# MaxChen228/pingpong-selfplay-ai

Hardware: AMD Instinct MI355X
Metric: env-steps/sec (whole node) at 65536 arenas, 1/2/4/8 GPUs; CPU-ref baseline (higher is better)
Workload: dtype f64 env state / f32 QNet; 1 GPU; configs[2]: 65536 arenas/GPU, full DQN train_iterative loop (act both players + env tick + PER push/sample + double-DQN update + Adam + target sync); arenas_per_gpu=65536, global_arenas=65536, pool=8, batch=256, updates_per_vector_step=1, memory_size=1000000, parallelism=dp1 (arena shards, 1 all-reduce/update)

## Files before the change

### pingpong-selfplay-ai_amd/csrc/pm_mfma.h

```cpp
#pragma once
#include "pm_dev.h"

namespace pm {

typedef float f32x16 __attribute__((ext_vector_type(16)));
typedef float f32x4v16 __attribute__((ext_vector_type(4)));
typedef __attribute__((address_space(3))) void lds_void;

constexpr int PLAIN = 4936;
enum : int {
    F_W1 = 0,
    F_W2 = 512,
    F_B1 = 4608,
    F_B2 = 4672,
    F_H = 4736,
    F_BH = 4992,
    F_SIZE = 5008,
};
static_assert(PLAIN + F_SIZE == PM_QNET_NW, "effective weight block size");

__device__ __forceinline__ int rho(int r) { return (r & 3) + 8 * (r >> 2); }

__device__ __forceinline__ float relu(float x) { return __int_as_float(max(__float_as_int(x), 0)); }

__device__ __forceinline__ void write_feature_frag_image(const float* __restrict__ p, float* __restrict__ f) {
    const int t = threadIdx.x, nt = blockDim.x;
    for (int k = t; k < 512; k += nt) {
        const int jt = k >> 8, lane = (k >> 2) & 63, s = k & 3;
        const int row = 32 * jt + (lane & 31), kk = 2 * s + (lane >> 5);
        f[F_W1 + k] = kk == 0 ? p[B1 + row] : p[W1 + row * 7 + kk - 1];
    }
    for (int k = t; k < 4096; k += nt) {
        const int e = k & 3, lane = (k >> 2) & 63, rq = (k >> 8) & 3, tt = (k >> 10) & 1, jt = k >> 11;
        const int row = 32 * jt + (lane & 31), col = 32 * tt + rho(4 * rq + e) + 4 * (lane >> 5);
        f[F_W2 + k] = p[W2 + row * 64 + col];
    }
    for (int k = t; k < 64; k += nt) {
        const int r = k & 15, h = (k >> 4) & 1, jt = k >> 5;
        f[F_B1 + k] = p[B1 + 32 * jt + rho(r) + 4 * h];
        f[F_B2 + k] = p[B2 + 32 * jt + rho(r) + 4 * h];
    }
}
__device__ __forceinline__ void write_feature_frags(const float* __restrict__ p, float* __restrict__ w) {
    for (int k = threadIdx.x; k < PM_QNET_HEAD_OFF; k += blockDim.x) w[k] = p[k];
    write_feature_frag_image(p, w + PLAIN);
}

__device__ __forceinline__ void write_head_frags(const float* heads, float* __restrict__ w) {
    const int t = threadIdx.x, nt = blockDim.x;
    for (int k = t; k < 260; k += nt) w[WH + k] = heads[k];
    float* f = w + PLAIN;
    for (int k = t; k < 256; k += nt) {
        const int c = k & 3, r = (k >> 2) & 15, tt = (k >> 6) & 1, h = k >> 7;
        f[F_H + k] = heads[c * 64 + 32 * tt + rho(r) + 4 * h];
    }
    if (t < 16) f[F_BH + t] = t < 4 ? heads[256 + t] : 0.f;
}

constexpr int kLwChunks = (F_SIZE / 4 + 63) / 64;
constexpr int kLwFloats = kLwChunks * 256;

template <int N>
__device__ __forceinline__ void copy_lds_f32(const float* __restrict__ src, float* dst) {
    const int wv = threadIdx.x >> 6, lane = threadIdx.x & 63, nw = blockDim.x >> 6;
    for (int c = wv; c * 64 < N; c += nw) {
        const int k = min(c * 64 + lane, N - 1);
        __builtin_amdgcn_global_load_lds((const void*)(src + k), (lds_void*)(dst + c * 64), 4, 0, 0);
    }
}
constexpr int pad64(int n) { return (n + 63) / 64 * 64; }
template <int N>
__device__ __forceinline__ void copy_lds_f32x4(const float* __restrict__ src, float* dst) {
    static_assert(N % 4 == 0, "whole float4s");
    const int wv = threadIdx.x >> 6, lane = threadIdx.x & 63, nw = blockDim.x >> 6;
    const float4* s4 = reinterpret_cast<const float4*>(src);
    for (int c = wv; c * 256 < N; c += nw) {
        const int k = min(c * 64 + lane, N / 4 - 1);
        __builtin_amdgcn_global_load_lds((const void*)(s4 + k), (lds_void*)(dst + c * 256), 16, 0, 0);
    }
}
constexpr int pad256(int n) { return (n + 255) / 256 * 256; }

__device__ __forceinline__ void stage_frags_lds(const float* __restrict__ w, float* lw, int rot) {
    const int wv = threadIdx.x >> 6, lane = threadIdx.x & 63, nw = blockDim.x >> 6;
    const float4* src = reinterpret_cast<const float4*>(w + PLAIN);
    float4* lw4 = reinterpret_cast<float4*>(lw);
    rot %= kLwChunks;
    for (int c0 = wv; c0 < kLwChunks; c0 += nw) {
        const int c = c0 + rot < kLwChunks ? c0 + rot : c0 + rot - kLwChunks;
        const int k = min(c * 64 + lane, F_SIZE / 4 - 1);
        __builtin_amdgcn_global_load_lds((const void*)(src + k), (lds_void*)(lw4 + c * 64), 16, 0, 0);
    }
}

constexpr int kListNets = 64;
constexpr int kListBlock = 256;
struct OppListSmem {
    int woff[kListBlock / 64][kListNets];
    int noff[kListNets], ncnt[kListNets];
};
__device__ __forceinline__ void write_opp_lists(int nn, int32_t* opp_list, int32_t* opp_cnt, OppListSmem& sm, int blk,
                                                int i, bool valid, int net) {
    if (nn > kListNets) return;
    const int lane = threadIdx.x & 63, wv = threadIdx.x >> 6;
    int rank = 0;
    for (int k = 0; k < nn; ++k) {
        const bool m = valid && net == k;
        const unsigned long long b = __ballot(m);
        if (m) rank = __popcll(b & ((1ull << lane) - 1ull));
        if (lane == 0) sm.woff[wv][k] = __popcll(b);
    }
    __syncthreads();
    if (wv == 0) {
        int acc = 0;
        if (lane < nn) {
            for (int w = 0; w < kListBlock / 64; ++w) {
                const int c = sm.woff[w][lane];
                sm.woff[w][lane] = acc;
                acc += c;
            }
        }
        const int inc = wave_incl_scan_i32(acc);
        if (lane < nn) { sm.ncnt[lane] = acc; sm.noff[lane] = inc - acc; }
    }
    __syncthreads();
    if (valid) opp_list[(size_t)blk * kListBlock + sm.noff[net] + sm.woff[wv][net] + rank] = i;
    if ((int)threadIdx.x < nn) opp_cnt[(size_t)blk * nn + threadIdx.x] = (sm.noff[threadIdx.x] << 16) | sm.ncnt[threadIdx.x];
}

__device__ __forceinline__ void compact_load(const int32_t* __restrict__ id, int lo, int hi, int (&v)[16]) {
    const int base = lo + 16 * (int)threadIdx.x;
    if (base + 16 <= hi && (reinterpret_cast<uintptr_t>(id + base) & 15) == 0) {
        const int4* p4 = reinterpret_cast<const int4*>(id + base);
#pragma unroll
        for (int q = 0; q < 4; ++q) {
            const int4 x = p4[q];
            v[4 * q] = x.x; v[4 * q + 1] = x.y; v[4 * q + 2] = x.z; v[4 * q + 3] = x.w;
        }
    } else {
#pragma unroll
        for (int r = 0; r < 16; ++r) v[r] = base + r < hi ? id[base + r] : -1;
    }
}
__device__ __forceinline__ void compact_scan(const int (&v)[16], int net, int lo, int* list, int* count, int* wtot) {
    const int t = threadIdx.x, lane = t & 63, wv = t >> 6, nw = blockDim.x >> 6;
    const int base = lo + 16 * t;
    unsigned mask = 0;
#pragma unroll
    for (int r = 0; r < 16; ++r) mask |= (v[r] == net ? 1u : 0u) << r;
    const int c = __popc(mask);
    const int incl = wave_incl_scan_i32(c);
    if (lane == 63) wtot[wv] = incl;
    __syncthreads();
    int off = 0, total = 0;
    for (int w = 0; w < nw; ++w) {
        off += w < wv ? wtot[w] : 0;
        total += wtot[w];
    }
    int p = off + incl - c;
    while (mask) {
        const int r = __ffs(mask) - 1;
        mask &= mask - 1;
        list[p++] = base + r;
    }
    if (t == 0) *count = total;
}

struct TileOut {
    int8_t* act;
    float* q;
    double eps;
    uint64_t seed, ctr;
};

__device__ __forceinline__ void heads_to_frags(const float* heads, float* hf) {
    for (int k = threadIdx.x; k < 260; k += blockDim.x) {
        if (k < 256) {
            const int c = k & 3, r = (k >> 2) & 15, tt = (k >> 6) & 1, h = k >> 7;
            hf[k] = heads[c * 64 + 32 * tt + rho(r) + 4 * h];
        } else {
            hf[k] = heads[k];
        }
    }
}

__device__ __forceinline__ void tile_hidden_h1(const float* lw, const float (&xs)[4], int lane, f32x16 (&c1)[2],
                                               f32x16 (&c2)[2]) {
    const int h = lane >> 5;
    const f32x16 zero = {};
#pragma unroll
    for (int jt = 0; jt < 2; ++jt) {
        const float4 w = reinterpret_cast<const float4*>(lw + F_W1)[jt * 64 + lane];
        c1[jt] = __builtin_amdgcn_mfma_f32_32x32x2f32(w.x, xs[0], zero, 0, 0, 0);
        c1[jt] = __builtin_amdgcn_mfma_f32_32x32x2f32(w.y, xs[1], c1[jt], 0, 0, 0);
        c1[jt] = __builtin_amdgcn_mfma_f32_32x32x2f32(w.z, xs[2], c1[jt], 0, 0, 0);
        c1[jt] = __builtin_amdgcn_mfma_f32_32x32x2f32(w.w, xs[3], c1[jt], 0, 0, 0);
    }
#pragma unroll
    for (int jt = 0; jt < 2; ++jt)
#pragma unroll
        for (int r = 0; r < 16; ++r) c1[jt][r] = relu(c1[jt][r]);
    const float4* w2 = reinterpret_cast<const float4*>(lw + F_W2) + lane;
#pragma unroll
    for (int jt = 0; jt < 2; ++jt) {
        const float4* b = reinterpret_cast<const float4*>(lw + F_B2 + (jt * 2 + h) * 16);
#pragma unroll
        for (int q4 = 0; q4 < 4; ++q4) {
            const float4 v = b[q4];
            c2[jt][4 * q4 + 0] = v.x; c2[jt][4 * q4 + 1] = v.y; c2[jt][4 * q4 + 2] = v.z; c2[jt][4 * q4 + 3] = v.w;
        }
    }
    float4 wcur = w2[0];
#pragma unroll
    for (int g8 = 0; g8 < 16; ++g8) {
        const int jt = g8 >> 3, t = (g8 >> 2) & 1, rq = g8 & 3;
        const float4 wnext = w2[((g8 + 1) & 15) * 64];
        c2[jt] = __builtin_amdgcn_mfma_f32_32x32x2f32(wcur.x, c1[t][4 * rq + 0], c2[jt], 0, 0, 0);
        c2[jt] = __builtin_amdgcn_mfma_f32_32x32x2f32(wcur.y, c1[t][4 * rq + 1], c2[jt], 0, 0, 0);
        c2[jt] = __builtin_amdgcn_mfma_f32_32x32x2f32(wcur.z, c1[t][4 * rq + 2], c2[jt], 0, 0, 0);
        c2[jt] = __builtin_amdgcn_mfma_f32_32x32x2f32(wcur.w, c1[t][4 * rq + 3], c2[jt], 0, 0, 0);
        wcur = wnext;
        __builtin_amdgcn_sched_barrier(0);
    }
}
__device__ __forceinline__ void tile_hidden(const float* lw, const float (&xs)[4], int lane, f32x16 (&c2)[2]) {
    f32x16 c1[2];
    tile_hidden_h1(lw, xs, lane, c1, c2);
}

__device__ __forceinline__ void tile_heads(const float* hf, const f32x16 (&c2)[2], int lane, float (&q)[3]) {
    const int h = lane >> 5;
    float v = 0.f, a0 = 0.f, a1 = 0.f, a2 = 0.f;
    const float4* hw = reinterpret_cast<const float4*>(hf + h * 128);
#pragma unroll
    for (int t = 0; t < 2; ++t) {
#pragma unroll
        for (int r = 0; r < 16; ++r) {
            const float x = relu(c2[t][r]);
            const float4 w = hw[t * 16 + r];
            v = fmaf(w.x, x, v);
            a0 = fmaf(w.y, x, a0);
            a1 = fmaf(w.z, x, a1);
            a2 = fmaf(w.w, x, a2);
        }
        __builtin_amdgcn_sched_barrier(0);
    }
    v += __shfl_xor(v, 32);
    a0 += __shfl_xor(a0, 32);
    a1 += __shfl_xor(a1, 32);
    a2 += __shfl_xor(a2, 32);
    v += hf[256];
    a0 += hf[257];
    a1 += hf[258];
    a2 += hf[259];
    const float mean = ((a0 + a1) + a2) / 3.0f;
    q[0] = v + (a0 - mean);
    q[1] = v + (a1 - mean);
// ... 375 lines not shown
```

### pingpong-selfplay-ai_amd/csrc/pm_per.h

```cpp
#pragma once
#include <hip/hip_runtime.h>
#include <stdint.h>

#include "pongmi.h"
#include "pm_dev.h"

namespace pm {

constexpr int PER_SUB = 64;
constexpr int PER_FAN = 16;
constexpr int PER_CHUNK = PER_SUB * PER_FAN;

__host__ __device__ inline int64_t per_pad(int64_t n_doubles) { return ((n_doubles * 8 + 255) / 256) * 256; }

struct PerTree {
    double* chunk;
    double* sub;
    float* leaf;
    int64_t nchunk, nsub;
};

__host__ __device__ inline PerTree per_tree(void* work, int64_t cap) {
    PerTree t;
    t.nsub = (cap + PER_SUB - 1) / PER_SUB;
// ... 131 lines not shown
        int64_t d = d0 + i;
        if (d >= pr.cap) d -= pr.cap;
        acc += lo + i < pr.cap ? (double)(d < pr.n ? pr.pval : v[i]) : 0.0;
    }
    return acc;
}
__device__ __forceinline__ double per_combine(double q0, double q1, double q2, double q3) {
    return ((q0 + q1) + q2) + q3;
}
__device__ __forceinline__ double per_sub_sum(const float* __restrict__ leaf, int64_t sb, const PushRange pr) {
    const double q0 = per_quarter(leaf, sb, 0, pr), q1 = per_quarter(leaf, sb, 1, pr);
    const double q2 = per_quarter(leaf, sb, 2, pr), q3 = per_quarter(leaf, sb, 3, pr);
    return per_combine(q0, q1, q2, q3);
}
__device__ __forceinline__ double per_sub_sum4(const float* __restrict__ leaf, int64_t sb, const PushRange pr) {
    const int lane = threadIdx.x & 63;
    const double q = per_quarter(leaf, sb, lane & 3, pr);
    return per_combine(quad_f64<0>(q), quad_f64<1>(q), quad_f64<2>(q), quad_f64<3>(q));
}

__device__ __forceinline__ bool per_sub_pushed(int64_t sb, const PushRange pr) {
    const int64_t lo = sb * PER_SUB;
    return lo + PER_SUB <= pr.cap && pr.dist(lo) + PER_SUB <= pr.n;
}
__device__ __forceinline__ double per_sub_pushed_sum(const PushRange pr) {
    double q = 0.0;
#pragma unroll
    for (int i = 0; i < 16; ++i) q += (double)pr.pval;
    return per_combine(q, q, q, q);
}

__device__ __forceinline__ double per_chunk_sum(const PerTree& t, int64_t c) {
    double v[PER_FAN];
#pragma unroll
    for (int k = 0; k < PER_FAN; ++k) v[k] = c * PER_FAN + k < t.nsub ? t.sub[c * PER_FAN + k] : 0.0;
    double acc = 0.0;
#pragma unroll
    for (int k = 0; k < PER_FAN; ++k) acc += v[k];
    return acc;
}

__device__ __forceinline__ void per_nodes_block(const PerTree& tr, const PushRange& pr, double* subl) {
    const int64_t sb = (int64_t)blockIdx.x * 64 + (threadIdx.x >> 2);
    const double v = per_sub_sum4(tr.leaf, sb < tr.nsub ? sb : tr.nsub - 1, pr);
    if ((threadIdx.x & 3) == 0) {
        subl[threadIdx.x >> 2] = sb < tr.nsub ? v : 0.0;
        if (sb < tr.nsub) tr.sub[sb] = v;
    }
    __syncthreads();
    const int64_t c = (int64_t)blockIdx.x * 4 + threadIdx.x;
    if (threadIdx.x < 4 && c < tr.nchunk) {
        double acc = 0.0;
#pragma unroll
        for (int k = 0; k < PER_FAN; ++k) acc += subl[threadIdx.x * PER_FAN + k];
        tr.chunk[c] = acc;
    }
}

constexpr int PER_BS = 64;
constexpr int PER_ROUND = 1024;

struct PerSampleSmem {
    double incl[PER_ROUND];
    double wsum[4];
};

__device__ inline double per_round_prefix(const double (&v)[4], double base, PerSampleSmem& sm) {
    const int t = threadIdx.x, lane = t & 63, wv = t >> 6;
    double run[4], acc = 0.0;
#pragma unroll
    for (int e = 0; e < 4; ++e) { acc += v[e]; run[e] = acc; }
    const double incl = wave_incl_scan_dpp(acc, lane);
    const double excl = wave_shr1_f64(incl);
    if (lane == 63) sm.wsum[wv] = incl;
    __syncthreads();
    double wb = base;
    for (int w = 0; w < wv; ++w) wb += sm.wsum[w];
    const double ex = wb + excl;
#pragma unroll
    for (int e = 0; e < 4; ++e) sm.incl[4 * t + e] = ex + run[e];
    const double tot = ((base + sm.wsum[0]) + sm.wsum[1]) + sm.wsum[2] + sm.wsum[3];
    __syncthreads();
    return tot;
}

__device__ __forceinline__ int per_lds_search(const PerSampleSmem& sm, int n, double x) {
    static_assert(PER_ROUND == 1024, "per_lds_search's five base-4 digits");
    int base = 0;
#pragma unroll
    for (int stride = 256; stride >= 1; stride >>= 2) {
        const int np = stride == 256 ? 4 : 3;
        double v[4];
#pragma unroll
        for (int i = 0; i < np; ++i) v[i] = sm.incl[min(base + stride * (i + 1) - 1, n - 1)];
        int cnt = 0;
#pragma unroll
        for (int i = 0; i < np; ++i) cnt += (base + stride * (i + 1) - 1 < n && !(v[i] > x)) ? 1 : 0;
        base += stride * cnt;
    }
    return base;
}

template <int NV>
__device__ __forceinline__ int per_group_find(const double (&v)[NV], double x, double& before, double& val) {
    const int lane = threadIdx.x & 63, q = lane & 3, g0 = lane & ~3;
    double acc = 0.0;
#pragma unroll
    for (int e = 0; e < NV; ++e) acc += v[e];
    const double s0 = quad_f64<0>(acc), s1 = quad_f64<1>(acc), s2 = quad_f64<2>(acc);
    const double ex = q == 0 ? 0.0 : (q == 1 ? s0 : (q == 2 ? s0 + s1 : (s0 + s1) + s2));
    double pre[NV + 1];
    pre[0] = ex;
#pragma unroll
    for (int e = 0; e < NV; ++e) pre[e + 1] = pre[e] + v[e];
    int k = -1;
    double hb = 0.0, hv = 0.0;
#pragma unroll
    for (int e = NV - 1; e >= 0; --e) {
        const bool h = pre[e + 1] > x;
        k = h ? e : k;
        hb = h ? pre[e] : hb;
        hv = h ? v[e] : hv;
    }
    const unsigned gh = (unsigned)(__ballot(k >= 0) >> g0) & 15u;
    int src;
    if (gh) {
        src = __ffs(gh) - 1;
    } else {
        hb = ex;
        hv = 0.0;
#pragma unroll
        for (int e = 0; e < NV; ++e) {
            const bool z = v[e] > 0.0;
            k = z ? e : k;
            hb = z ? pre[e] : hb;
            hv = z ? v[e] : hv;
        }
        const unsigned gn = (unsigned)(__ballot(k >= 0) >> g0) & 15u;
        src = gn ? 31 - __clz(gn) : 0;
        k = k < 0 ? 0 : k;
    }
    const int kk = quad_sel_i32(k, src);
    before = quad_sel_f64(hb, src);
    val = quad_sel_f64(hv, src);
    return src * NV + kk;
}

struct NoHook {
    __device__ void operator()() const {}
};
__device__ __forceinline__ float per_is_weight(int64_t size, double pa, double total, double beta) {
    return (float)pow((double)size * (pa / total), -beta);
}
template <bool RAW = false, class UFn, class OutFn, class Hook = NoHook>
__device__ inline void per_sample_block(bool active, int64_t size, const PerTree& tr, const PushRange& pr, double beta,
                                        int j0, int bs, PerSampleSmem& sm, UFn ufn, OutFn out, Hook l2done = Hook()) {
    const int t = threadIdx.x, q = t & 3;
    const int j = j0 + (t >> 2);
    const bool one_round = tr.nchunk <= PER_ROUND;
    double vc[4] = {0.0, 0.0, 0.0, 0.0};
    if (one_round) {
#pragma unroll
        for (int e = 0; e < 4; ++e) {
            const int64_t c = 4 * t + e;
            vc[e] = c < tr.nchunk ? tr.chunk[c] : 0.0;
        }
        asm volatile("" ::"v"(vc[0]), "v"(vc[1]), "v"(vc[2]), "v"(vc[3]));
    }
    if (!active) return;
    const int64_t nb = (size + PER_CHUNK - 1) / PER_CHUNK;
    const double u = j < bs ? ufn(j) : 0.0;
    double total = 0.0;
    if (nb > PER_ROUND) {
        for (int64_t c0 = 0; c0 < nb; c0 += PER_ROUND) {
            double v[4];
#pragma unroll
            for (int e = 0; e < 4; ++e) {
                const int64_t c = c0 + 4 * t + e;
                v[e] = c < nb ? tr.chunk[c] : 0.0;
            }
            total = per_round_prefix(v, total, sm);
        }
    }
    int64_t blk = -1, lastnz = 0;
    double before = 0.0, lastbef = 0.0, x = 0.0, run = 0.0;
    for (int64_t c0 = 0; c0 < nb; c0 += PER_ROUND) {
        double v[4];
#pragma unroll
        for (int e = 0; e < 4; ++e) {
            const int64_t c = c0 + 4 * t + e;
            v[e] = c < nb ? (one_round ? vc[e] : tr.chunk[c]) : 0.0;
        }
        const double end = per_round_prefix(v, run, sm);
        if (nb <= PER_ROUND) total = end;
        x = u * total;
        const int n = (int)(nb - c0 < PER_ROUND ? nb - c0 : PER_ROUND);
        if (blk < 0 && end > run) {
            const int k = per_lds_search(sm, n, x);
            if (k < n) {
                blk = c0 + k;
                before = k ? sm.incl[k - 1] : run;
            } else {
                int lo = 0, hi = n - 1;
                while (lo < hi) {
                    const int mid = (lo + hi) >> 1;
                    if (sm.incl[mid] >= sm.incl[n - 1]) hi = mid;
                    else lo = mid + 1;
                }
                lastnz = c0 + lo;
                lastbef = lo ? sm.incl[lo - 1] : run;
            }
        }
        run = end;
        __syncthreads();
    }
    if (blk < 0) { blk = lastnz; before = lastbef; }
    PM_BLK(4);
    l2done();
    double sv[4];
    const int64_t s0 = blk * PER_FAN + 4 * q;
#pragma unroll
    for (int e = 0; e < 4; ++e) sv[e] = s0 + e < tr.nsub ? tr.sub[s0 + e] : 0.0;
    double b1, v1;
    const int64_t sb = blk * PER_FAN + per_group_find<4>(sv, x - before, b1, v1);
    PM_BLK(5);
    double lv[16];
    {
        const int64_t lo = sb * PER_SUB + 16 * q;
        float f[16];
        if (lo + 16 <= pr.cap) {
            const float4* p4 = reinterpret_cast<const float4*>(tr.leaf + lo);
#pragma unroll
            for (int k = 0; k < 4; ++k) {
                const float4 a = p4[k];
                f[4 * k] = a.x; f[4 * k + 1] = a.y; f[4 * k + 2] = a.z; f[4 * k + 3] = a.w;
            }
        } else {
#pragma unroll
            for (int k = 0; k < 16; ++k) f[k] = lo + k < pr.cap ? tr.leaf[lo + k] : 0.f;
        }
        const int64_t d0 = pr.dist(lo);
        const int64_t wrap = pr.cap - d0;
        const int kw = (int)(wrap < 0 ? 0 : (wrap < 16 ? wrap : 16));
        const int ka = min(kw, (int)(pr.n - d0 < 0 ? 0 : (pr.n - d0 < 16 ? pr.n - d0 : 16)));
        const int kb = (int)(wrap + pr.n < 0 ? 0 : (wrap + pr.n < 16 ? wrap + pr.n : 16));
        const int ks = (int)(size - lo < 0 ? 0 : (size - lo < 16 ? size - lo : 16));
#pragma unroll
        for (int k = 0; k < 16; ++k) {
            const bool cov = k < ka || (k >= kw && k < kb);
            const double lf = (double)(cov ? pr.pval : f[k]);
            lv[k] = k < ks ? lf : 0.0;
        }
    }
    double b0, pa;
    const int k = per_group_find<16>(lv, x - before - b1, b0, pa);
    PM_BLK(6);
    if (q == 0 && j < bs) {
        if constexpr (RAW) out(j, sb * PER_SUB + k, pa, total);
        else out(j, sb * PER_SUB + k, per_is_weight(size, pa, total, beta));
    }
    PM_BLK(7);
}

int per_launch_build(const float* prios, int64_t cap, float alpha, const pm_ctrl* ctrl, int64_t n_push, void* work,
                     hipStream_t st);
int per_launch_update(float* prios, const int64_t* idx, const float* err, int bs, hipStream_t st);
int per_launch_nodes(void* work, int64_t cap, hipStream_t st);

}
```

### pingpong-selfplay-ai_amd/csrc/pm_sp_rollout.hip

```cpp
#include "pm_sp.h"

#ifdef PM_DIAG
static __device__ unsigned long long pm_diag_env[8][1024];
#define PM_ENV_STAMP(k, blk)                                                                   \
    do {                                                                                       \
        asm volatile("" ::: "memory");                                                         \
        if (threadIdx.x == 0 && (blk) < 1024) pm_diag_env[(k)][(blk)] = __builtin_amdgcn_s_memrealtime(); \
    } while (0)
#define PM_ENV_STAMP_DRAIN(k, blk)                                                             \
    do {                                                                                       \
        asm volatile("s_waitcnt vmcnt(0) lgkmcnt(0)" ::: "memory");                            \
        if (threadIdx.x == 0 && (blk) < 1024) pm_diag_env[(k)][(blk)] = __builtin_amdgcn_s_memrealtime(); \
    } while (0)
#else
#define PM_ENV_STAMP(k, blk) \
    do {                     \
    } while (0)
#define PM_ENV_STAMP_DRAIN(k, blk) \
    do {                           \
    } while (0)
#endif

namespace {
__device__ __forceinline__ bool learner_active(const pm_selfplay& sp) {
    const int64_t s = sp.ctrl->size + sp.n;
    return (s < sp.cap ? s : sp.cap) >= sp.batch;
}
}

__device__ __forceinline__ void sample_block(const pm_selfplay& sp, int b, bool pending, PerSampleSmem& sm) {
    const pm_ctrl* c = sp.ctrl;
    const int64_t s = c->size + sp.n;
    const int64_t size = s < sp.cap ? s : sp.cap;
    const int64_t frame = c->frame_idx + 1;
    const PushRange pr = pending ? push_of(sp, c->pos, c->size, c->max_prio) : PushRange{0, 0, sp.cap, 0.f};
    const uint64_t key = sp.seed_env;
    per_sample_block(
        size >= sp.batch, size, per_tree(sp.per_work, sp.cap), pr, beta_of(sp, frame), b * PER_BS,
        min(sp.batch, b * PER_BS + PER_BS), sm,
        [&](int j) {
            const U4 r = philox64((uint32_t)j, TAG_PER, (uint64_t)frame, key);
            return u53(r.x, r.y);
        },
        [&](int j, int64_t idx, float w) {
            sp.idx[j] = idx;
            sp.isw[j] = w;
        });
}

#ifndef PM_ENV_WT
#define PM_ENV_WT 7
#endif
constexpr bool kEnvWTRows = (PM_ENV_WT & 1) != 0, kEnvWTState = (PM_ENV_WT & 2) != 0, kEnvWTObs = (PM_ENV_WT & 4) != 0;
constexpr bool kEnvWTPrio = (PM_ENV_WT & 8) != 0;
constexpr bool kEnvWTFrow = (PM_ENV_WT & 16) != 0;

__device__ __forceinline__ bool gb_current(const pm_selfplay& sp) {
    return sp.featB && sp.gB && sp.gB_ready && !sp.frow;
}

__device__ __forceinline__ void env_fwd_block(const pm_selfplay& sp, int f, bool pending = true) {
    __shared__ __attribute__((aligned(16))) float lw[kLwFloats];
    __shared__ __attribute__((aligned(16))) float hf[2][264];
    if (!learner_active(sp)) return;
    stage_frags_lds(sp.w_B, lw, f * 5);
    for (int k = threadIdx.x; k < 2 * 264; k += blockDim.x) hf[k / 264][k % 264] = sp.learn_heads[k];
    __syncthreads();
    const int lane = threadIdx.x & 63, B = sp.batch;
    const int r0 = f * 128 + (int)(threadIdx.x >> 6) * 32;
    if (r0 >= 2 * B) return;
    const int r = min(r0 + (lane & 31), 2 * B - 1);
    const bool nxt = r >= B;
    const int j = nxt ? r - B : r;
    const int64_t id = sp.idx[j];
    const pm_ctrl* c = sp.ctrl;
    const bool mine = r0 + (lane & 31) < 2 * B && !(pending && push_of(sp, c->pos, c->size, c->max_prio).covers(id));
    f32x16 c2[2];
    float qb[3], qt[3];
    float rb[2];
    batch_row_fwd(sp, lw, hf[0], hf[1], id, nxt, lane, c2, qb, qt, rb);
    if (mine) store_hfeat(sp.hfeat, j, nxt, lane, c2, qb, qt, rb);
}

union ActSpShared {
    ActShared act;
    PerSampleSmem per;
};
__global__ __launch_bounds__(kActBlock, 4) void k_act_sp(const pm_selfplay sp, int part) {
    __shared__ __attribute__((aligned(16))) ActSpShared sh;
    PM_BLK(0);
    const int nsb = part == PM_ACT_A ? 0 : (sp.batch + PER_BS - 1) / PER_BS;
    {
        const ActGrid g{sp.n, sp.n_pool + 1, sp.chunk_A, sp.chunk_P, part == PM_ACT_A ? 0 : 1};
        const int fb = (int)blockIdx.x - nsb - g.blocks();
        if (fb >= 0) {
            const int t0 = fb * kFeatTilesAct;
            feat_tiles(sh.act.lw, sp.w_B, sp.obsB, sp.n, t0, min(t0 + kFeatTilesAct, feat_ntiles(sp.n)), sp.featB);
            return;
        }
    }
    if ((int)blockIdx.x < nsb) {
        PM_STAMP(64);
        sample_block(sp, (int)blockIdx.x, true, sh.per);
        PM_STAMP(65);
        PM_BLK_END();
        return;
    }
    if ((int)blockIdx.x == nsb) PM_STAMP_ANY(70);
    const ActGrid g{sp.n, sp.n_pool + 1, sp.chunk_A, sp.chunk_P, part == PM_ACT_A ? 0 : 1};
    const TileOut outA{sp.aA, nullptr, -1.0, 0, 0};
    const TileOut outB{sp.aB, nullptr, -1.0, 0, 0};
    act_block(sh.act, g, sp.w_opp, sp.n_pool > 0 ? sp.opp : nullptr, sp.w_B, sp.obsA, sp.obsB, outA, outB,
              (int)blockIdx.x - nsb, sp.n_pool + 1 <= kListNets ? sp.opp_list : nullptr, sp.opp_cnt);
    PM_BLK_END();
}

constexpr int kSampBlock = 8;
struct SampleFwd16Smem {
    PerSampleSmem per;
    int64_t sidx[kSampBlock];
    __attribute__((aligned(16))) float h1s[4][4][16][4];
    __attribute__((aligned(16))) float c2s[2][8][16][4];
    __attribute__((aligned(16))) float hf[pad256(2 * 264)];
    __attribute__((aligned(16))) float opw[2][2][4][32];
};
__device__ __forceinline__ void sample_fwd_block16(const pm_selfplay& sp, int b, SampleFwd16Smem& sm) {
    constexpr int NS = kSampBlock;
    const pm_ctrl* c = sp.ctrl;
    const int64_t csize = c->size, cpos = c->pos, cframe = c->frame_idx;
    const float cmaxp = c->max_prio;
    const int64_t s = csize + sp.n;
    const int64_t size = s < sp.cap ? s : sp.cap;
    const int64_t frame = cframe + 1;
    const bool active = size >= sp.batch;
    const PushRange pr = push_of(sp, cpos, csize, cmaxp);
    const double beta = beta_of(sp, frame);
    const uint64_t key = sp.seed_env;
    const int lane = threadIdx.x & 63, col = lane & 15, g = lane >> 4;
    const int rt = __builtin_amdgcn_readfirstlane(threadIdx.x >> 6);
    int wj = -1;
    double wpa = 0.0, wtot = 1.0;
    float4 f1 = make_float4(0.f, 0.f, 0.f, 0.f), f2[8], b2r = f1;
#pragma unroll
    for (int m = 0; m < 8; ++m) f2[m] = f1;
    per_sample_block<true>(
        active, size, per_tree(sp.per_work, sp.cap), pr, beta, b * NS, min(sp.batch, b * NS + NS), sm.per,
        [&](int j) {
            const U4 r = philox64((uint32_t)j, TAG_PER, (uint64_t)frame, key);
            return u53(r.x, r.y);
        },
        [&](int j, int64_t idx, double pa, double total) {
            sp.idx[j] = idx;
            sm.sidx[j - b * NS] = idx;
            wj = j;
            wpa = pa;
            wtot = total;
        },
        [&] {
            const float* w = sp.w_B;
            const int jt = rt >> 1, fl = 32 * (g & 1) + 16 * (rt & 1) + col;
            f1 = reinterpret_cast<const float4*>(w + PLAIN + F_W1)[jt * 64 + fl];
            const float4* q2 = reinterpret_cast<const float4*>(w + PLAIN + F_W2) + jt * 8 * 64 + fl;
#pragma unroll
            for (int m = 0; m < 8; ++m) f2[m] = q2[m * 64];
            b2r = *reinterpret_cast<const float4*>(w + B2 + 16 * rt + 4 * g);
            copy_lds_f32x4<2 * 264>(sp.learn_heads, sm.hf);
        });
    if (!active) return;
    __syncthreads();
    PM_BLK(1);
    const int B = sp.batch;
    const bool nxt = col >= NS;
    const int j = b * NS + (col & (NS - 1));
    const int64_t id = sm.sidx[min(j, B - 1) - b * NS];
    const bool mine = j < B && !pr.covers(id);
    const float* tr = sp.trans + id * PM_TRANS_F;
    const float* o = tr + (nxt ? 8 : 0);
    const float o0 = o[g == 0 ? 0 : g - 1];
    const float x1 = o[3 + g];
    const float rb0 = tr[7], rb1 = tr[15];
    if (rt >= 2) heads_to_opw(sm.opw, rt - 2, sm.hf + (rt - 2) * 264);
    float wisw = 0.f;
    if (wj >= 0) wisw = per_is_weight(size, wpa, wtot, beta);
    const bool odd = (g >> 1) != 0;
    const float w1r[2] = {odd ? f1.y : f1.x, odd ? f1.w : f1.z};
    float w2r[16];
#pragma unroll
    for (int m = 0; m < 8; ++m) {
        w2r[2 * m] = odd ? f2[m].y : f2[m].x;
        w2r[2 * m + 1] = odd ? f2[m].w : f2[m].z;
    }
    {
        const float x0 = g == 0 ? 1.0f : o0;
        const f32x4v16 zero = {0.f, 0.f, 0.f, 0.f};
        f32x4v16 c1 = __builtin_amdgcn_mfma_f32_16x16x4f32(w1r[0], x0, zero, 0, 0, 0);
        c1 = __builtin_amdgcn_mfma_f32_16x16x4f32(w1r[1], x1, c1, 0, 0, 0);
#pragma unroll
        for (int r = 0; r < 4; ++r) {
            const int q = l2_pos(16 * rt + 4 * g + r), sq = q >> 2;
            sm.h1s[q & 3][sq >> 2][col][sq & 3] = relu(c1[r]);
        }
    }
    __syncthreads();
    float hw4[32];
    {
        const float* src = sm.opw[lane >> 5][(lane >> 4) & 1][lane & 3];
#pragma unroll
        for (int k = 0; k < 8; ++k) {
            const float4 w = *reinterpret_cast<const float4*>(src + 4 * k);
            hw4[4 * k] = w.x; hw4[4 * k + 1] = w.y; hw4[4 * k + 2] = w.z; hw4[4 * k + 3] = w.w;
        }
    }
    const float4 bhr = *reinterpret_cast<const float4*>(sm.hf + (lane >> 5) * 264 + 256);
    float bs[16];
#pragma unroll
    for (int k = 0; k < 4; ++k) {
        const float4 v = *reinterpret_cast<const float4*>(sm.h1s[g][k][col]);
        bs[4 * k] = v.x; bs[4 * k + 1] = v.y; bs[4 * k + 2] = v.z; bs[4 * k + 3] = v.w;
    }
    f32x4v16 c2 = {b2r.x, b2r.y, b2r.z, b2r.w};
#pragma unroll
    for (int i = 0; i < 16; ++i) c2 = __builtin_amdgcn_mfma_f32_16x16x4f32(w2r[i], bs[i], c2, 0, 0, 0);
    float* row = sp.hfeat + (size_t)j * 80;
#pragma unroll
    for (int r = 0; r < 4; ++r) {
        const int u = 16 * rt + 4 * g + r, q = head_pos(u);
        c2[r] = relu(c2[r]);
        sm.c2s[(u >> 2) & 1][q >> 2][col][q & 3] = c2[r];
    }
    if (mine && !nxt) *reinterpret_cast<float4*>(row + 16 * rt + 4 * g) = make_float4(c2[0], c2[1], c2[2], c2[3]);
    __syncthreads();
    if (rt != 0) return;
    if (wj >= 0) sp.isw[wj] = wisw;
    const int set = lane >> 5, hh = (lane >> 4) & 1;
    float xb[32];
#pragma unroll
    for (int k = 0; k < 8; ++k) {
        const float4 x = *reinterpret_cast<const float4*>(sm.c2s[hh][k][col]);
        xb[4 * k] = x.x; xb[4 * k + 1] = x.y; xb[4 * k + 2] = x.z; xb[4 * k + 3] = x.w;
    }
    f32x4v16 acc = {0.f, 0.f, 0.f, 0.f};
#pragma unroll
    for (int q = 0; q < 32; ++q) acc = __builtin_amdgcn_mfma_f32_4x4x1f32(hw4[q], xb[q], acc, 0, 0, 0);
    float v = xor16_sum(acc[0]), a0 = xor16_sum(acc[1]), a1 = xor16_sum(acc[2]), a2 = xor16_sum(acc[3]);
    v += bhr.x;
    a0 += bhr.y;
    a1 += bhr.z;
    a2 += bhr.w;
    const float mean = ((a0 + a1) + a2) / 3.0f;
    const float q0 = v + (a0 - mean), q1 = v + (a1 - mean), q2 = v + (a2 - mean);
    if (mine && hh == 0) {
        if (set == 0) {
            float* qd = row + (nxt ? 68 : 64);
            qd[0] = q0; qd[1] = q1; qd[2] = q2;
            if (!nxt) {
                row[67] = rb0;
                row[71] = rb1;
            }
        } else if (nxt) {
            row[72] = q0; row[73] = q1; row[74] = q2;
        }
    }
}

__device__ __forceinline__ void write_opp_lists(const pm_selfplay& sp, OppListSmem& sm, int blk, int i, bool valid,
                                                int net) {
    write_opp_lists(sp.n_pool + 1, sp.opp_list, sp.opp_cnt, sm, blk, i, valid, net);
}

struct EnvSmem {
    float lds[2][kBlock][7];
    float4 rows[kBlock][4];
    long long red[kBlock / 64][6];
    OppListSmem ol;
};
struct ActEnvSmem {
    EnvSmem e;
    float lw[kLwFloats];
};

template <bool ACT>
__device__ __forceinline__ void env_block(const pm_selfplay& sp, int blk, EnvSmem& sm, float* lw) {
    const int i0 = blk * kBlock;
    const int i = i0 + threadIdx.x;
    const int lane = threadIdx.x & 63, wv = threadIdx.x >> 6;
    const bool valid = i < sp.n;
    const int ii = valid ? i : sp.n - 1;
    const pm_ctrl* c = sp.ctrl;
    if (blk == 0) PM_STAMP_ANY(72);
    PM_ENV_STAMP(0, blk);
    float xs[2][4];
    f32x16 fc2[2][2];
    const bool ahead = ACT && gb_current(sp);
    if (ahead) {
    } else if (ACT && sp.featB) {
        if (threadIdx.x < 65)
            reinterpret_cast<float4*>(lw + F_H)[threadIdx.x] =
                reinterpret_cast<const float4*>(sp.w_B + PLAIN + F_H)[threadIdx.x];
        const int tlast = feat_ntiles(sp.n) - 1;
#pragma unroll
        for (int k = 0; k < 2; ++k) feat_load(sp.featB, min(blk * 8 + 2 * wv + k, tlast), lane, fc2[k]);
    } else if (ACT) {
        stage_frags_lds(sp.w_B, lw, blk);
#pragma unroll
        for (int k = 0; k < 2; ++k) {
            const int row = min(i0 + 64 * wv + 32 * k + (lane & 31), sp.n - 1);
            tile_inputs(sp.obsB + (size_t)row * 7, lane >> 5, xs[k]);
        }
    }
    const uint32_t ns = (uint32_t)__builtin_nontemporal_load(&sp.st.serves[ii]);
    const int64_t pos = c->pos, size = c->size;
    const float cmaxp = c->max_prio;
    const uint64_t cstep = c->step;
    const double ceps = c->epsilon;
    const int o = sp.opp[ii];
    const float er0 = sp.ep_reward[ii];
    Arena a = load_arena(sp.st, ii);
    const int aA = sp.aA[ii];
    int aB = ACT ? (ahead ? (int)sp.gB[ii] : 0) : sp.aB[ii];
    __builtin_amdgcn_sched_barrier(0);
    const float maxp = push_prio(size, cmaxp);
    float* leaf = per_tree(sp.per_work, sp.cap).leaf;
    const float pval = prio_pow(maxp, (float)sp.alpha);

    int onext, eps_a;
    bool eps_hit;
    double svx, svy, sspn;
    {
        const U4 rr = philox64((uint32_t)ii, TAG_ACT, cstep, sp.seed_env);
        eps_hit = u53(rr.x, rr.y) < ceps;
        eps_a = (int)below(rr.z, 3u);
        const U4 q = philox((uint32_t)ii, TAG_OPP, ns, 0u, sp.seed_env);
        onext = (sp.n_pool > 0 && u53(q.x, q.y) < sp.pool_ratio) ? 1 + below(q.z, (uint32_t)sp.n_pool) : 0;
        philox_serve(sp.env, (uint32_t)ii, ns, sp.seed_env, svx, svy, sspn);
        asm volatile("" ::"v"(onext), "v"(svx), "v"(svy), "v"(sspn), "v"(eps_hit), "v"(eps_a));
        __builtin_amdgcn_sched_barrier(0);
    }
    if (ahead) {
        const unsigned long long fb = __ballot(valid && aB == PM_GB_NONE);
        if (fb) {
#pragma unroll
            for (int k = 0; k < 2; ++k) {
                if (!(uint32_t)(fb >> (32 * k))) continue;
                float q[3];
                feat_load(sp.featB, blk * 8 + 2 * wv + k, lane, fc2[k]);
                tile_heads(sp.w_B + PLAIN + F_H, fc2[k], lane, q);
                if ((lane >> 5) == k) aB = argmax3(q);
            }
        }
        if (!valid) aB = 0;
        PM_ENV_STAMP(7, blk);
    } else if (ACT) {
        __syncthreads();
        PM_ENV_STAMP(7, blk);
        int act[2];
#pragma unroll
        for (int k = 0; k < 2; ++k) {
            float q[3];
            if (sp.featB) {
                tile_heads(lw + F_H, fc2[k], lane, q);
            } else {
                f32x16 c2[2];
                tile_hidden(lw, xs[k], lane, c2);
                tile_heads(lw + F_H, c2, lane, q);
            }
            act[k] = argmax3(q);
            if (sp.featB && sp.frow) {
                const int ar = i0 + 64 * wv + 32 * k + (lane & 31);
                if (ar < sp.n) {
                    int64_t slot = pos + ar;
                    if (slot >= sp.cap) slot -= sp.cap;
                    float4* fr = reinterpret_cast<float4*>(sp.frow + slot * 64) + (lane >> 5);
#pragma unroll
                    for (int jt = 0; jt < 2; ++jt)
#pragma unroll
                        for (int q4 = 0; q4 < 4; ++q4)
                            st_f4<kEnvWTFrow>(fr + 8 * jt + 2 * q4,
                                              make_float4(relu(fc2[k][jt][4 * q4]), relu(fc2[k][jt][4 * q4 + 1]),
                                                          relu(fc2[k][jt][4 * q4 + 2]), relu(fc2[k][jt][4 * q4 + 3])));
                }
            }
        }
        aB = lane < 32 ? act[0] : act[1];
    }
    PM_ENV_STAMP(1, blk);
    if (eps_hit) aB = eps_a;
    float oA[7], oB[7];
    observe(a, oA, oB);
    float rA, rB;
    const int d = tick(sp.env, a, aA, aB, rA, rB);
    float nA[7], nB[7];
    observe(a, nA, nB);
#ifdef PM_DIAG
    asm volatile("" ::"v"(nA[0]), "v"(nB[1]), "v"(d));
#endif
    PM_ENV_STAMP(2, blk);
    const float er = er0 + rB;
    const bool fin = valid && d;
    {
        const bool win = er > 0.f;
        const unsigned long long mf = __ballot(fin), mA = __ballot(fin && o == 0), mwA = __ballot(fin && o == 0 && win);
        const unsigned long long mP = __ballot(fin && o != 0), mwP = __ballot(fin && o != 0 && win);
        const int rs = wave_sum(fin ? (int)er : 0);
        if (lane == 0) {
            sm.red[wv][0] = __popcll(mf); sm.red[wv][1] = __popcll(mA); sm.red[wv][2] = __popcll(mwA);
            sm.red[wv][3] = __popcll(mP); sm.red[wv][4] = __popcll(mwP); sm.red[wv][5] = rs;
        }
    }
    int onew = o;
    {
        static_assert(PM_TRANS_F == 16, "store_ring_rows16 writes 64-byte rows");
        const float4 piece[4] = {make_float4(oB[0], oB[1], oB[2], oB[3]), make_float4(oB[4], oB[5], oB[6], rB),
                                 make_float4(nB[0], nB[1], nB[2], nB[3]),
                                 make_float4(nB[4], nB[5], nB[6], __int_as_float(aB | (d << 8)))};
        store_ring_rows16<kEnvWTRows>(sp.trans, pos, sp.cap, i0 + 64 * wv, sp.n, sm.rows + 64 * wv, piece);
    }
    if (valid) {
        int64_t slot = pos + i;
        if (slot >= sp.cap) slot -= sp.cap;
        st_out<kEnvWTPrio>(&sp.prios[slot], maxp);
        st_out<kEnvWTPrio>(&leaf[slot], pval);
        float ernew = er;
        if (d) {
            onew = onext;
            serve(a, svx, svy, sspn);
            sp.st.serves[i] = (int32_t)ns + 1;
            ernew = 0.f;
            observe(a, nA, nB);
        }
        store_arena<kEnvWTState>(sp.st, i, a);
        sp.opp[i] = onew;
        sp.aB[i] = (int8_t)aB;
        sp.ep_reward[i] = ernew;
    }
    PM_ENV_STAMP(3, blk);
#pragma unroll
    for (int k = 0; k < 7; ++k) { sm.lds[0][threadIdx.x][k] = nA[k]; sm.lds[1][threadIdx.x][k] = nB[k]; }
    __syncthreads();
    PM_ENV_STAMP(4, blk);
    if (threadIdx.x < 6) {
        long long t = 0;
        for (int w = 0; w < kBlock / 64; ++w) t += sm.red[w][threadIdx.x];
        sp.partials[(size_t)blk * 8 + threadIdx.x] = t;
    }
    write_opp_lists(sp, sm.ol, blk, i, valid, onew);
    PM_ENV_STAMP(5, blk);
    copy_rows7<kEnvWTObs>(sp.obsA, sm.lds[0], i0, sp.n);
    copy_rows7<kEnvWTObs>(sp.obsB, sm.lds[1], i0, sp.n);
    PM_ENV_STAMP_DRAIN(6, blk);
}

__global__ __launch_bounds__(kBlock) void k_env(const pm_selfplay sp) {
    const int blk = (int)blockIdx.x;
    const int nenv = (sp.n + kBlock - 1) / kBlock;
    if (blk >= nenv) {
        env_fwd_block(sp, blk - nenv);
        return;
    }
    __shared__ __attribute__((aligned(16))) EnvSmem sm;
    env_block<false>(sp, blk, sm, nullptr);
}

union ActEnvShared {
    ActEnvSmem ae;
    SampleFwd16Smem sf16;
};
__global__ __launch_bounds__(kBlock) void k_actenv(const pm_selfplay sp) {
    __shared__ __attribute__((aligned(16))) ActEnvShared sh;
    const int nsb = (sp.batch + kSampBlock - 1) / kSampBlock;
    if ((int)blockIdx.x < nsb) {
        PM_BLK(0);
        sample_fwd_block16(sp, (int)blockIdx.x, sh.sf16);
        PM_BLK_END();
        return;
    }
    env_block<true>(sp, (int)blockIdx.x - nsb, sh.ae.e, sh.ae.lw);
}

__global__ __launch_bounds__(kBlock) void k_sp_init(const pm_selfplay sp) {
    __shared__ __attribute__((aligned(16))) float lds[kBlock][7];
    const int i0 = blockIdx.x * kBlock;
    const int i = i0 + threadIdx.x;
    float oA[7] = {0}, oB[7] = {0};
    int net = 0;
    if (i < sp.n) {
        const uint32_t ns = (uint32_t)sp.st.serves[i];
        const U4 q = philox((uint32_t)i, TAG_OPP, ns, 0u, sp.seed_env);
        net = (sp.n_pool > 0 && u53(q.x, q.y) < sp.pool_ratio) ? 1 + below(q.z, (uint32_t)sp.n_pool) : 0;
        sp.opp[i] = net;
        Arena a;
        double vx, vy, spn;
        philox_serve(sp.env, (uint32_t)i, ns, sp.seed_env, vx, vy, spn);
        serve(a, vx, vy, spn);
        store_arena(sp.st, i, a);
        sp.st.serves[i] = (int32_t)ns + 1;
        sp.ep_reward[i] = 0.f;
        observe(a, oA, oB);
    }
    {
        __shared__ OppListSmem ol;
        write_opp_lists(sp, ol, blockIdx.x, i, i < sp.n, net);
    }
    store_rows7(sp.obsA, lds, oA, i0, sp.n);
    store_rows7(sp.obsB, lds, oB, i0, sp.n);
}

__global__ __launch_bounds__(256) void k_resample(const pm_selfplay sp) {
    __shared__ PerSampleSmem sm;
    sample_block(sp, (int)blockIdx.x, false, sm);
}
__global__ __launch_bounds__(kBlock) void k_batch_fwd(const pm_selfplay sp) { env_fwd_block(sp, (int)blockIdx.x, false); }

namespace {
int launch_act(const pm_selfplay* sp, int part, hipStream_t st) {
    const ActGrid g{sp->n, sp->n_pool + 1, sp->chunk_A, sp->chunk_P, part == PM_ACT_A ? 0 : 1};
    const int nsb = part == PM_ACT_A ? 0 : (sp->batch + PER_BS - 1) / PER_BS;
    int blocks = part == PM_ACT_B ? nsb + g.nb() : nsb + g.blocks();
    if (part != PM_ACT_B && sp->featB) blocks += (feat_ntiles(sp->n) + kFeatTilesAct - 1) / kFeatTilesAct;
    hipLaunchKernelGGL(k_act_sp, dim3(blocks), dim3(kActBlock), 0, st, *sp, part);
    PM_LAUNCHED("k_act_sp");
    return PM_OK;
}
}

int pm::selfplay_launch_init(const pm_selfplay* sp, hipStream_t st) {
    hipLaunchKernelGGL(k_sp_init, dim3(pm_blocks(sp->n, kBlock)), dim3(kBlock), 0, st, *sp);
    PM_LAUNCHED("k_sp_init");
    return PM_OK;
}

extern "C" int pm_selfplay_act(const pm_selfplay* sp, void* stream) {
    return pm_selfplay_act_part(sp, PM_ACT_ALL, stream);
}

extern "C" int pm_selfplay_act_part(const pm_selfplay* sp, int32_t part, void* stream) {
    int rc = selfplay_check(sp);
    if (rc) return rc;
    PM_REQUIRE(part == PM_ACT_ALL || part == PM_ACT_B || part == PM_ACT_A, PM_E_ARG,
               "pm_selfplay_act_part: part=%d", part);
    return launch_act(sp, part, pm_stream(stream));
}

extern "C" int pm_selfplay_env(const pm_selfplay* sp, void* stream) {
    int rc = selfplay_check(sp);
    if (rc) return rc;
    const unsigned nfwd = pm_blocks(2 * sp->batch, 128);
    hipLaunchKernelGGL(k_env, dim3(pm_blocks(sp->n, kBlock) + nfwd), dim3(kBlock), 0, pm_stream(stream), *sp);
    PM_LAUNCHED("k_env");
    return PM_OK;
}

extern "C" int pm_selfplay_actenv(const pm_selfplay* sp, void* stream) {
    int rc = selfplay_check(sp);
    if (rc) return rc;
    const unsigned nsb = pm_blocks(sp->batch, kSampBlock);
    pm_launch(PM_TIMER_ACTENV, k_actenv, dim3(nsb + pm_blocks(sp->n, kBlock)), dim3(kBlock), pm_stream(stream), *sp);
    PM_LAUNCHED("k_actenv");
    return PM_OK;
}

extern "C" int pm_selfplay_rollout(const pm_selfplay* sp, void* stream) {
    int rc = pm_selfplay_act(sp, stream);
    return rc ? rc : pm_selfplay_env(sp, stream);
}

extern "C" int pm_selfplay_resample(const pm_selfplay* sp, void* stream) {
    int rc = selfplay_check(sp);
    if (rc) return rc;
    hipStream_t st = pm_stream(stream);
    hipLaunchKernelGGL(k_resample, dim3((sp->batch + PER_BS - 1) / PER_BS), dim3(256), 0, st, *sp);
    PM_LAUNCHED("k_resample");
    hipLaunchKernelGGL(k_batch_fwd, dim3(pm_blocks(2 * sp->batch, 128)), dim3(kBlock), 0, st, *sp);
    PM_LAUNCHED("k_batch_fwd");
    return PM_OK;
}

#ifdef PM_DIAG
extern "C" int pm_diag_read_sp_rollout(uint64_t* out, int32_t n) {
    hipError_t e = hipMemcpyFromSymbol(out, HIP_SYMBOL(pm_diag_buf), sizeof(uint64_t) * (n < 256 ? n : 256));
    return e == hipSuccess ? 0 : (int)e;
}
extern "C" int pm_diag_clear_sp_rollout(void) {
    static const unsigned long long z[256] = {0};
    return (int)hipMemcpyToSymbol(HIP_SYMBOL(pm_diag_buf), z, sizeof(z));
}
extern "C" int pm_diag_read_blk(uint64_t* out) {
    return (int)hipMemcpyFromSymbol(out, HIP_SYMBOL(pm_diag_blk), sizeof(uint64_t) * 8 * 4096);
}
extern "C" int pm_diag_read_env(uint64_t* out) {
    return (int)hipMemcpyFromSymbol(out, HIP_SYMBOL(pm_diag_env), sizeof(uint64_t) * 8 * 1024);
}
#endif
```

Baseline: 2.352 billion env-steps/s.

## Pack opponent-list counts for small net pools and split PER sample hooks

Adds a fast path in write_opp_lists for up to 16 nets. Per-net counts are packed into bytes of four ints, so one set of wave scans, one barrier and a DPP prefix scan replace a per-net ballot loop followed by a second scan phase. The PER sampler hook is split in two: the weight-fragment loads are issued after the sub-level loads, and the LDS copy of the heads after the leaf loads, with sched_barriers fixing the order, to overlap global latency. A diagnostic CU-placement stamp is also added, but it only compiles under PM_DIAG.

Result: faster. 2.388 billion env-steps/s (median of 6 runs) (+1.5%).

```diff
diff --git a/pingpong-selfplay-ai_amd/csrc/pm_mfma.h b/pingpong-selfplay-ai_amd/csrc/pm_mfma.h
--- a/pingpong-selfplay-ai_amd/csrc/pm_mfma.h
+++ b/pingpong-selfplay-ai_amd/csrc/pm_mfma.h
@@ -95,14 +95,49 @@
 
 constexpr int kListNets = 64;
 constexpr int kListBlock = 256;
-struct OppListSmem {
-    int woff[kListBlock / 64][kListNets];
+constexpr int kListPacked = 16;
+struct alignas(16) OppListSmem {
+    union {
+        int woff[kListBlock / 64][kListNets];
+        int wtot[kListPacked / 4][kListBlock / 64];
+    };
     int noff[kListNets], ncnt[kListNets];
 };
 __device__ __forceinline__ void write_opp_lists(int nn, int32_t* opp_list, int32_t* opp_cnt, OppListSmem& sm, int blk,
                                                 int i, bool valid, int net) {
     if (nn > kListNets) return;
     const int lane = threadIdx.x & 63, wv = threadIdx.x >> 6;
+    if (nn <= kListPacked) {
+        static_assert(kListBlock / 64 == 4 && kListPacked == 16, "four waves' totals as one int4, nets 0-15 in a row");
+        const bool m = valid && (unsigned)net < (unsigned)nn;
+        const int sh = 8 * (net & 3), wsel = net >> 2;
+        const int one = m ? 1 << sh : 0;
+        int s[4];
+#pragma unroll
+        for (int j = 0; j < 4; ++j) s[j] = wave_incl_scan_i32(wsel == j ? one : 0);
+        if (lane == 63) {
+#pragma unroll
+            for (int j = 0; j < 4; ++j) sm.wtot[j][wv] = s[j];
+        }
+        const int mine = wsel == 0 ? s[0] : (wsel == 1 ? s[1] : (wsel == 2 ? s[2] : s[3]));
+        const int rank = ((mine >> sh) & 255) - 1;
+        __syncthreads();
+        const int k = lane & 15, ks = 8 * (k & 3);
+        const int4 t = *reinterpret_cast<const int4*>(sm.wtot[k >> 2]);
+        const int c0 = (t.x >> ks) & 255, c1 = (t.y >> ks) & 255, c2 = (t.z >> ks) & 255, c3 = (t.w >> ks) & 255;
+        const int cnt = (c0 + c1) + (c2 + c3);
+        const int pre = wv == 0 ? 0 : (wv == 1 ? c0 : (wv == 2 ? c0 + c1 : c0 + c1 + c2));
+        int inc = cnt;
+        inc += __builtin_amdgcn_update_dpp(0, inc, 0x111, 0xF, 0xF, true);
+        inc += __builtin_amdgcn_update_dpp(0, inc, 0x112, 0xF, 0xF, true);
+        inc += __builtin_amdgcn_update_dpp(0, inc, 0x114, 0xF, 0xF, true);
+        inc += __builtin_amdgcn_update_dpp(0, inc, 0x118, 0xF, 0xF, true);
+        const int noff = inc - cnt;
+        const int base = __shfl(noff + pre, net & (kListPacked - 1));
+        if (m) opp_list[(size_t)blk * kListBlock + base + rank] = i;
+        if ((int)threadIdx.x < nn) opp_cnt[(size_t)blk * nn + threadIdx.x] = (noff << 16) | cnt;
+        return;
+    }
     int rank = 0;
     for (int k = 0; k < nn; ++k) {
         const bool m = valid && net == k;
diff --git a/pingpong-selfplay-ai_amd/csrc/pm_per.h b/pingpong-selfplay-ai_amd/csrc/pm_per.h
--- a/pingpong-selfplay-ai_amd/csrc/pm_per.h
+++ b/pingpong-selfplay-ai_amd/csrc/pm_per.h
@@ -307,9 +307,10 @@
 __device__ __forceinline__ float per_is_weight(int64_t size, double pa, double total, double beta) {
     return (float)pow((double)size * (pa / total), -beta);
 }
-template <bool RAW = false, class UFn, class OutFn, class Hook = NoHook>
+template <bool RAW = false, class UFn, class OutFn, class Hook1 = NoHook, class Hook0 = NoHook>
 __device__ inline void per_sample_block(bool active, int64_t size, const PerTree& tr, const PushRange& pr, double beta,
-                                        int j0, int bs, PerSampleSmem& sm, UFn ufn, OutFn out, Hook l2done = Hook()) {
+                                        int j0, int bs, PerSampleSmem& sm, UFn ufn, OutFn out, Hook1 l1issued = Hook1(),
+                                        Hook0 l0issued = Hook0()) {
     const int t = threadIdx.x, q = t & 3;
     const int j = j0 + (t >> 2);
     const bool one_round = tr.nchunk <= PER_ROUND;
@@ -371,11 +372,13 @@
     }
     if (blk < 0) { blk = lastnz; before = lastbef; }
     PM_BLK(4);
-    l2done();
     double sv[4];
     const int64_t s0 = blk * PER_FAN + 4 * q;
 #pragma unroll
     for (int e = 0; e < 4; ++e) sv[e] = s0 + e < tr.nsub ? tr.sub[s0 + e] : 0.0;
+    __builtin_amdgcn_sched_barrier(0);
+    l1issued();
+    __builtin_amdgcn_sched_barrier(0);
     double b1, v1;
     const int64_t sb = blk * PER_FAN + per_group_find<4>(sv, x - before, b1, v1);
     PM_BLK(5);
@@ -394,6 +397,9 @@
 #pragma unroll
             for (int k = 0; k < 16; ++k) f[k] = lo + k < pr.cap ? tr.leaf[lo + k] : 0.f;
         }
+        __builtin_amdgcn_sched_barrier(0);
+        l0issued();
+        __builtin_amdgcn_sched_barrier(0);
         const int64_t d0 = pr.dist(lo);
         const int64_t wrap = pr.cap - d0;
         const int kw = (int)(wrap < 0 ? 0 : (wrap < 16 ? wrap : 16));
diff --git a/pingpong-selfplay-ai_amd/csrc/pm_sp_rollout.hip b/pingpong-selfplay-ai_amd/csrc/pm_sp_rollout.hip
--- a/pingpong-selfplay-ai_amd/csrc/pm_sp_rollout.hip
+++ b/pingpong-selfplay-ai_amd/csrc/pm_sp_rollout.hip
@@ -12,7 +12,17 @@
         asm volatile("s_waitcnt vmcnt(0) lgkmcnt(0)" ::: "memory");                            \
         if (threadIdx.x == 0 && (blk) < 1024) pm_diag_env[(k)][(blk)] = __builtin_amdgcn_s_memrealtime(); \
     } while (0)
+static __device__ unsigned long long pm_diag_env_place[1024];
+#define PM_ENV_PLACE(blk)                                                                      \
+    do {                                                                                       \
+        if (threadIdx.x == 0 && (blk) < 1024)                                                  \
+            pm_diag_env_place[(blk)] =                                                         \
+                (unsigned long long)__smid() | ((unsigned long long)(__builtin_amdgcn_s_getreg(20 | (3 << 11)) & 15) << 16); \
+    } while (0)
 #else
+#define PM_ENV_PLACE(blk) \
+    do {                  \
+    } while (0)
 #define PM_ENV_STAMP(k, blk) \
     do {                     \
     } while (0)
@@ -164,8 +174,8 @@
 #pragma unroll
             for (int m = 0; m < 8; ++m) f2[m] = q2[m * 64];
             b2r = *reinterpret_cast<const float4*>(w + B2 + 16 * rt + 4 * g);
-            copy_lds_f32x4<2 * 264>(sp.learn_heads, sm.hf);
-        });
+        },
+        [&] { copy_lds_f32x4<2 * 264>(sp.learn_heads, sm.hf); });
     if (!active) return;
     __syncthreads();
     PM_BLK(1);
@@ -289,6 +299,7 @@
     const pm_ctrl* c = sp.ctrl;
     if (blk == 0) PM_STAMP_ANY(72);
     PM_ENV_STAMP(0, blk);
+    PM_ENV_PLACE(blk);
     float xs[2][4];
     f32x16 fc2[2][2];
     const bool ahead = ACT && gb_current(sp);
@@ -590,4 +601,7 @@
 extern "C" int pm_diag_read_env(uint64_t* out) {
     return (int)hipMemcpyFromSymbol(out, HIP_SYMBOL(pm_diag_env), sizeof(uint64_t) * 8 * 1024);
 }
+extern "C" int pm_diag_read_env_place(uint64_t* out) {
+    return (int)hipMemcpyFromSymbol(out, HIP_SYMBOL(pm_diag_env_place), sizeof(uint64_t) * 1024);
+}
 #endif
```
